# atonderski/future-object-detection

Hardware: AMD Instinct MI355X
Metric: frame-sequences/sec fwd+bwd, T=6 900x1600 (higher is better)
Workload: dtype bf16; 1 GPU; spatiotemporal ConditionalDETR (ResNet-50, 6 enc + 6 dec layers, 128 queries), T=6 frames 900x1600, batch 2/GPU, num_images K=5 (5 past frames live), random-init weights; step = forward (incl. Hungarian set loss, post-proc, AP bookkeeping) + backward + clip + AdamW; global_batch=2, frames=6, num_images=5, parallelism=dp1

## Files before the change

future-object-detection_amd/csrc/api.cpp:

```cpp
#include <stdarg.h>
#include <stdio.h>
#include <stdlib.h>
#include <string.h>

#include <mutex>

#include "../../include/fod.h"
#include "knobs.h"

static thread_local char g_err[512] = "";

void fod_set_error(const char* fmt, ...) {
  va_list ap;
  va_start(ap, fmt);
  vsnprintf(g_err, sizeof(g_err), fmt, ap);
  va_end(ap);
}

extern "C" size_t fod_last_error(char* buf, size_t cap) {
  const size_t n = strlen(g_err);
  if (buf && cap) {
    const size_t c = n < cap - 1 ? n : cap - 1;
    memcpy(buf, g_err, c);
    buf[c] = 0;
  }
  return n;
}

extern "C" int fod_abi_version(void) { return FOD_ABI_VERSION; }

extern "C" size_t fod_workspace_bytes(int kind) {
  switch (kind) {
    case FOD_WS_NT_SPLIT: return (size_t)FOD_NT_SPLIT_WS_FLOATS * sizeof(float);
    case FOD_WS_NT_SPLIT_TICKETS: return (size_t)FOD_NT_SPLIT_TICKETS * sizeof(unsigned);
    case FOD_WS_TN_PARTIALS: return FOD_TN_WS_BYTES;
    case FOD_WS_ATTN_SPLIT_PER_TILE: return (size_t)FOD_ATTN_SPLIT_WS_FLOATS_PER_TILE * sizeof(float);
    case FOD_WS_DET: return FOD_DET_WS_BYTES;
    case FOD_WS_TN_MULTI_DET: return FOD_TN_MULTI_DET_WS_BYTES;
    default: return 0;
  }
}

namespace {
struct KnobName {
  const char* name;
  int Knobs::*i;
  double Knobs::*d;
};
const KnobName KNOB_NAMES[] = {
    {"FOD_NT_SMALL", &Knobs::nt_small, nullptr},
    {"FOD_NT_NARROW", &Knobs::nt_narrow, nullptr},
    {"FOD_NT_SPLITK", &Knobs::nt_splitk, nullptr},
    {"FOD_NT_BIG", &Knobs::nt_big, nullptr},
    {"FOD_NT_BIG256", &Knobs::nt_big256, nullptr},
    {"FOD_NT_BIG_ILV", &Knobs::nt_big_ilv, nullptr},
    {"FOD_NT_BIG256_MINK", &Knobs::nt_big256_mink, nullptr},
    {"FOD_NT_BIG_MINK", &Knobs::nt_big_mink, nullptr},
    {"FOD_NT_BIG_MINN", &Knobs::nt_big_minn, nullptr},
    {"FOD_TN_SMALL", &Knobs::tn_small, nullptr},
    {"FOD_TN_BIG", &Knobs::tn_big, nullptr},
    {"FOD_TN_BIG_DENSE", &Knobs::tn_big_dense, nullptr},
    {"FOD_TN_BIG256", &Knobs::tn_big256, nullptr},
    {"FOD_TN_BIG_MIN", nullptr, &Knobs::tn_big_min},
    {"FOD_TN_BIG_SPLITS", &Knobs::tn_big_splits, nullptr},
    {"FOD_TN_WS", &Knobs::tn_ws, nullptr},
    {"FOD_TN_XCD", &Knobs::tn_xcd, nullptr},
    {"FOD_TN_ROWS", &Knobs::tn_rows, nullptr},
    {"FOD_ATTN_LDS", &Knobs::attn_lds, nullptr},
    {"FOD_ATTN_PF", &Knobs::attn_pf, nullptr},
    {"FOD_FP8_STAGE", &Knobs::fp8_stage, nullptr},
    {"FOD_LN_BWD_GROUPS", &Knobs::ln_bwd_groups, nullptr},
    {"FOD_BNK_VERSION", &Knobs::bnk_version, nullptr},
};

bool knob_parse(const KnobName& k, const char* text, Knobs& t) {
  char* end = nullptr;
  if (k.d) {
    const double v = strtod(text, &end);
    if (end == text || *end) return false;
    t.*k.d = v;
    return true;
  }
  if (Knobs{}.*k.i == Knobs::AUTO && !strcmp(text, "auto")) {
    t.*k.i = Knobs::AUTO;
    return true;
  }
  const long v = strtol(text, &end, 10);
  if (end == text || *end || v < 0 || v > 0x7FFFFFFF) return false;
  t.*k.i = (int)v;
  return true;
}

std::mutex g_knob_mutex;
Knobs& knob_table() {
  static Knobs table = [] {
    Knobs t;
    for (const KnobName& k : KNOB_NAMES)
      if (const char* text = getenv(k.name)) knob_parse(k, text, t);
    return t;
  }();
  return table;
}
const KnobName* knob_find(const char* name) {
  for (const KnobName& k : KNOB_NAMES)
    if (name && !strcmp(name, k.name)) return &k;
  fod_set_error("knob: unknown name %s", name ? name : "(null)");
  return nullptr;
}
}

Knobs fod_knobs() {
// ... 37 lines not shown
```

future-object-detection_amd/csrc/gemm_nt.hip:

```cpp
#include <stdlib.h>

#include <type_traits>

#include "common.h"
#include "gemm_nt.h"
#include "gemm_tn.h"

namespace {

using namespace fodnt;

template <typename T, int MODE, int NT, bool UTAP>
FOD_DEVINL void gemm_nt_body(const NtParams& p) {
  constexpr int VEC = Elem<T>::VEC;
  constexpr int BK = ROW_BYTES / (int)sizeof(T);
  constexpr int BN = 64 * NT;
  constexpr int KSTEPS = BK / 16;
  constexpr int BROWS = BN / 32;
  extern __shared__ __attribute__((aligned(16))) unsigned char smem[];
  unsigned char* sA = smem;
  unsigned char* sB = smem + 2 * BM * ROW_BYTES;

  const int tid = threadIdx.x;
  const int lane = tid & 63;
// ... 669 lines not shown
void fill_epilogue(NtParams& p, const fod_epilogue* e) {
  p.scale = e ? e->scale : nullptr;
  p.shift = e ? e->shift : nullptr;
  p.res = e ? e->residual : nullptr;
  p.ldr = e ? e->ld_residual : 0;
  p.res_row_mod = e ? e->residual_row_mod : 0;
  p.mask = e ? e->relu_mask : nullptr;
  p.ldmask = e ? e->ld_mask : 0;
  p.relu = e ? e->relu : 0;
  p.c_is_f32 = e ? e->out_f32 : 0;
  p.split_ws = e ? reinterpret_cast<float*>(e->split_ws) : nullptr;
  p.split_tickets = e ? reinterpret_cast<unsigned*>(e->split_tickets) : nullptr;
}

void decide_vec_epilogue(NtParams& p) {
  auto al = [](const void* q) { return ((uintptr_t)q % 16) == 0; };
  p.vec_epi = (p.N % 4 == 0) && (p.ldc % 4 == 0) && al(p.C) && (!p.scale || al(p.scale)) &&
              (!p.shift || al(p.shift)) && (!p.res || (p.ldr % 4 == 0 && al(p.res))) &&
              (!p.mask || (p.ldmask % 4 == 0 && al(p.mask)));
}

}

namespace fodnt {
namespace {
bool small_applies(int dtype, const NtParams& p, const Knobs& kn) {
  if (!kn.nt_small) return false;
  if (dtype != FOD_BF16 || !p.vec_epi) return false;
  const long blocks = (long)ceil_div(p.M, 64) * ceil_div(p.N, 64);
  if (blocks > 256) return false;
  if (p.res && ((long)(p.res_row_mod > 0 ? p.res_row_mod : p.M) * p.ldr + p.N) * 2 >= 0x7FFFFFF0L) return false;
  if (p.mask && ((long)p.M * p.ldmask + p.N) * 2 >= 0x7FFFFFF0L) return false;
  return true;
}

bool big256_applies(const NtParams& p, const Knobs& kn) {
  if (kn.nt_big256 == 0) return false;
  if (p.N < 256) return false;
  if (kn.nt_big256 == 2) return true;
  const long tiles = (long)ceil_div(p.M, BMB) * ceil_div(p.N, 256);
  return p.N % 256 == 0 && tiles >= 200;
}

bool big_applies(int mode, const NtParams& p, const Knobs& kn) {
  if (kn.nt_big == 0) return false;
  if (!p.vec_epi || p.a_seg_len || p.c_seg_cols) return false;
  if (mode == MODE_STEM) return false;
  if (mode != MODE_DENSE && (p.Cs % BKB_EL != 0 || p.K < BKB_EL)) return false;
  if (mode == MODE_DENSE && p.K % 8 != 0) return false;
  if (p.N % 4 != 0) return false;
  const long tiles = (long)ceil_div(p.M, BMB) * ceil_div(p.N, 128);
  if (kn.nt_big == 2) return true;
  if (mode != MODE_DENSE && p.K >= kn.nt_big256_mink && p.K < 1536 && big256_applies(p, kn)) return true;
  return p.K >= kn.nt_big_mink && p.N >= kn.nt_big_minn && tiles >= 200;
}
}

NtRoute route(int mode, int dtype, const NtParams& p, const Knobs& kn) {
  NtRoute r{};
  r.ksplit = 1;
  if (mode == MODE_DENSE && small_applies(dtype, p, kn)) {
    r.kernel = FOD_ROUTE_NT_SMALL;
    r.tile_n = 64;
    const long tiles = (long)ceil_div(p.N, 64) * ceil_div(p.M, 64);
    if (p.K >= 1024 && tiles <= 64 && kn.nt_splitk != 0) {
      const int cap = kn.nt_splitk > 1 ? (kn.nt_splitk < 8 ? kn.nt_splitk : 8) : 4;
      int ks = (int)(256 / tiles);
      if (ks > cap) ks = cap;
      if (ks > p.K / 256) ks = p.K / 256;
      r.wants_split_ws = ks > 1;
      if (ks > 1 && p.split_ws && p.split_tickets) r.ksplit = ks;
    }
    return r;
  }
  if (dtype == FOD_BF16 && big_applies(mode, p, kn)) {
    r.kernel = FOD_ROUTE_NT_BIG;
    const bool square = big256_applies(p, kn);
    r.tile_n = square ? 256 : 128;
    r.stages = square ? 2 : 3;
    r.interleave = kn.nt_big_ilv == Knobs::AUTO ? r.stages == 3 : kn.nt_big_ilv != 0;
    return r;
  }
  r.kernel = FOD_ROUTE_NT_128;
  r.stages = 2;
  const int narrow_below = kn.nt_narrow == Knobs::AUTO ? 320 : kn.nt_narrow;
  const long gy = ceil_div(p.M, BM);
  const long t_wide = gy * ceil_div(p.N, 128), t_narrow = gy * ceil_div(p.N, 64);
  const double fill_wide = (double)t_wide / (double)(ceil_div(t_wide, 512L) * 512L);
  const double fill_narrow = (double)t_narrow / (double)(ceil_div(t_narrow, 768L) * 768L);
  const bool narrow = p.N <= 64 || t_wide < narrow_below || (kn.nt_narrow == Knobs::AUTO && fill_narrow > 1.15 * fill_wide);
  r.tile_n = narrow ? 64 : 128;
  return r;
}
}

namespace {
int dense_params(NtParams& p, int dtype, const void* A, long lda, int a_row_mod, const void* B, long ldb, void* C,
                 long ldc, int M, int N, int K, const fod_epilogue* epi) {
  const int vec = dtype == FOD_BF16 ? 8 : 4;
  FOD_REQUIRE(M > 0 && N > 0 && K > 0, "gemm_nt: empty problem %d %d %d", M, N, K);
  FOD_REQUIRE(K % vec == 0 && lda % vec == 0 && ldb % vec == 0,
              "gemm_nt: K=%d lda=%ld ldb=%ld must be multiples of %d", K, lda, ldb, vec);
  FOD_REQUIRE(((uintptr_t)A % 16) == 0 && ((uintptr_t)B % 16) == 0, "gemm_nt: operands must be 16-byte aligned");
  p.A = A; p.B = B; p.C = C;
  p.lda = lda; p.ldb = ldb; p.ldc = ldc;
  p.M = M; p.N = N; p.K = K;
  p.a_row_mod = a_row_mod;
  fill_epilogue(p, epi);
  decide_vec_epilogue(p);
  const long esz = dtype == FOD_BF16 ? 2 : 4;
  const long a_rows = a_row_mod > 0 ? a_row_mod : M;
  const long ab = ((a_rows - 1) * lda + K) * esz, bb = ((long)(N - 1) * ldb + K) * esz;
  FOD_REQUIRE(ab < 0xFFFFFFF0L - 16 && bb < 0xFFFFFFF0L - 16, "gemm_nt: operand larger than 4 GiB");
  p.a_bytes = (unsigned)ab;
  p.b_bytes = (unsigned)bb;
  return FOD_OK;
}
}

extern "C" int fod_gemm_nt(int dtype, const void* A, long lda, int a_row_mod, const void* B, long ldb,
                           void* C, long ldc, int M, int N, int K, const fod_epilogue* epi,
                           hipStream_t stream) {
  FOD_REQUIRE(A && B && C, "gemm_nt: null operand");
  NtParams p{};
  if (int rc = dense_params(p, dtype, A, lda, a_row_mod, B, ldb, C, ldc, M, N, K, epi)) return rc;
  return launch<MODE_DENSE>(dtype, p, stream);
}

extern "C" int fod_gemm_nt_route(int dtype, long lda, int a_row_mod, long ldb, long ldc, int M, int N, int K,
                                 const fod_epilogue* epi, fod_nt_route* out) {
  FOD_REQUIRE(out && (dtype == FOD_BF16 || dtype == FOD_F32), "gemm_nt_route: bad args");
  NtParams p{};
  if (int rc = dense_params(p, dtype, nullptr, lda, a_row_mod, nullptr, ldb, nullptr, ldc, M, N, K, epi)) return rc;
// ... 228 lines not shown
```

future-object-detection_amd/csrc/gemm_nt_big.hip:

```cpp
#include <type_traits>

#include "common.h"
#include "gemm_nt.h"
#include "lds_dma.h"

namespace {

using namespace fodnt;

constexpr int A_DMA = BMB / 64;
template <int MODE, int BNB, int NSTAGE, bool ILV>
__global__ __launch_bounds__(512) void nt_big_kernel(const NtParams p) {
  constexpr int STAGE_BYTES = (BMB + BNB) * ROW_BYTES;
  constexpr int B_DMA = BNB / 64;
  constexpr int N_DMA = A_DMA + B_DMA;
  constexpr int NJ = BNB / 64;
  static_assert((BNB == 128 && NSTAGE == 3) || (BNB == 256 && NSTAGE == 2), "tile shapes: 256 x 128 x 3 stages, 256 x 256 x 2");
  typedef __bf16 T;
  constexpr unsigned ESZ = 2;
  constexpr unsigned BKB = BKB_EL * ESZ;
  constexpr int KSTEPS = BKB_EL / 16;
  extern __shared__ __attribute__((aligned(16))) unsigned char smem[];

  const int tid = threadIdx.x;
  const int lane = tid & 63;
  const int wave = __builtin_amdgcn_readfirstlane(tid >> 6);
  const int wm = wave >> 1, wn = wave & 1;
  const int xcd = blockIdx.x & 7, slot = blockIdx.x >> 3;
  const int nt_i = slot % p.gx;
  const int mt_i = (slot / p.gx) * 8 + xcd;
  if (mt_i >= p.gy) return;
  const int n0 = nt_i * BNB;
  const int m0 = mt_i * BMB;

  constexpr unsigned OOB = 0xFFFFFFF0u;
  const v4i rsA = make_rsrc(p.A, p.a_bytes), rsB = make_rsrc(p.B, p.b_bytes);
  const unsigned lds0 = (unsigned)(uintptr_t)(lds_ptr)smem;

  const int lrow = lane >> 3, lslot = lane & 7;
  unsigned a_base[A_DMA], a_cc[A_DMA];
  int a_h[A_DMA], a_w[A_DMA];
  int px_img = 0, px_h = 0, px_w = 0;
  if (MODE != MODE_DENSE) {
    const int mfirst = m0 + 8 * wave + lrow;
    const int hw = p.Hd * p.Wd;
    px_img = mfirst / hw;
    const int rem = mfirst - px_img * hw;
    px_h = rem / p.Wd;
    px_w = rem - px_h * p.Wd;
  }
#pragma unroll
  for (int i = 0; i < A_DMA; ++i) {
    const int row = 8 * (8 * i + wave) + lrow;
    const int m = m0 + row;
    const bool valid = m < p.M;
    a_cc[i] = (unsigned)((lslot ^ ((row >> 1) & 7)) * 16);
    if (MODE == MODE_DENSE) {
      const int r = p.a_row_mod > 0 ? (m % p.a_row_mod) : m;
      a_base[i] = valid ? (unsigned)((long)r * p.lda * (long)ESZ) + a_cc[i] : OOB;
      a_h[i] = a_w[i] = 0;
    } else {
      const int img = px_img, ph = px_h, pw = px_w;
      px_w += 64;
      while (px_w >= p.Wd) {
        px_w -= p.Wd;
        if (++px_h == p.Hd) {
          px_h = 0;
          ++px_img;
        }
      }
      a_base[i] = (unsigned)((long)img * p.Hs * p.Ws * p.Cs * (long)ESZ);
      if (MODE == MODE_CONV) {
        a_h[i] = valid ? ph * p.stride - p.pad : -(1 << 28);
        a_w[i] = pw * p.stride - p.pad;
      } else if (MODE == MODE_DGRAD_S2) {
        a_h[i] = valid ? ph + p.off_h : -(1 << 28);
        a_w[i] = pw + p.off_w;
      } else {
        a_h[i] = valid ? ph + p.pad : -(1 << 28);
        a_w[i] = pw + p.pad;
      }
      a_base[i] += ((unsigned)a_h[i] * (unsigned)p.Ws + (unsigned)a_w[i]) * (unsigned)p.Cs * ESZ + a_cc[i];
    }
  }
  unsigned b_base[B_DMA], b_cc[B_DMA];
#pragma unroll
  for (int i = 0; i < B_DMA; ++i) {
    const int row = 8 * (8 * i + wave) + lrow;
    const int n = n0 + row;
    b_cc[i] = (unsigned)((lslot ^ ((row >> 1) & 7)) * 16);
    b_base[i] = (n < p.N) ? (unsigned)((long)n * p.ldb * (long)ESZ) + b_cc[i] : OOB;
  }

  const int tap_w = MODE == MODE_DGRAD_S2 ? p.n_s : p.kw;
  const unsigned tap_row_skip = (unsigned)((p.Ws - tap_w) * p.Cs) * ESZ;
  const unsigned kb_row_skip = (unsigned)((2 * p.kw - 2 * tap_w) * p.Cs) * ESZ;
  const unsigned cs_b = (unsigned)p.Cs * ESZ;
  int tap_r = 0, tap_s = 0, tap_c = 0;
  unsigned tap_off = 0, tap_kb = 0;
  if (MODE == MODE_DGRAD_S2) tap_kb = (unsigned)((p.r_first * p.kw + p.s_first) * p.Cs) * ESZ;
  int next_kt = 0;

  struct TileCtx {
    int kt, r, s;
    unsigned kbyte, toff, kb, sA, sB;
// ... 27 lines not shown
    const bool tile_in = kt * BKB_EL < p.K;
    return TileCtx{kt, r, s, kbyte, toff, kb, sA, sB, tile_in};
  };
  auto issue_piece = [&](const TileCtx& c, auto pc_) {
    constexpr int pc = decltype(pc_)::value;
    if constexpr (pc < A_DMA) {
      constexpr int i = pc;
      unsigned off;
      if (MODE == MODE_DENSE) {
        const bool kin = (int)(c.kt * BKB_EL + (a_cc[i] >> 1)) < p.K;
        off = (kin && a_base[i] != OOB) ? a_base[i] + c.kbyte : OOB;
      } else {
        const int hs = MODE == MODE_CONV ? a_h[i] + c.r : a_h[i] - c.r;
        const int ws = MODE == MODE_CONV ? a_w[i] + c.s : a_w[i] - c.s;
        const bool ok = c.tile_in && (unsigned)hs < (unsigned)p.Hs && (unsigned)ws < (unsigned)p.Ws;
        off = ok ? (MODE == MODE_CONV ? a_base[i] + c.toff : a_base[i] - c.toff) : OOB;
      }
      dma16(rsA, c.sA + i * 8192, off);
    } else if constexpr (pc < A_DMA + B_DMA) {
      constexpr int i = pc - A_DMA;
      const bool kin = MODE == MODE_DENSE ? (int)(c.kt * BKB_EL + (b_cc[i] >> 1)) < p.K : c.tile_in;
      const unsigned off = (kin && b_base[i] != OOB) ? b_base[i] + c.kb : OOB;
      dma16(rsB, c.sB + i * 8192, off);
    }
  };
  auto issue_idx = [&](const TileCtx& c, int idx) {
    switch (idx) {
      case 0: issue_piece(c, std::integral_constant<int, 0>{}); break;
      case 1: issue_piece(c, std::integral_constant<int, 1>{}); break;
      case 2: issue_piece(c, std::integral_constant<int, 2>{}); break;
      case 3: issue_piece(c, std::integral_constant<int, 3>{}); break;
      case 4: issue_piece(c, std::integral_constant<int, 4>{}); break;
      case 5: issue_piece(c, std::integral_constant<int, 5>{}); break;
      case 6: issue_piece(c, std::integral_constant<int, 6>{}); break;
      case 7: issue_piece(c, std::integral_constant<int, 7>{}); break;
      default: break;
    }
  };
  auto issue_tile = [&](int stage) {
    const TileCtx c = begin_tile(stage);
#pragma unroll
    for (int idx = 0; idx < N_DMA; ++idx) issue_idx(c, idx);
  };

  f32x16 acc[2][NJ];
#pragma unroll
  for (int i = 0; i < 2; ++i)
#pragma unroll
    for (int j = 0; j < NJ; ++j)
#pragma unroll
      for (int r = 0; r < 16; ++r) acc[i][j][r] = 0.f;

  const int fr = lane & 31, fh = lane >> 5;
  auto read_frags = [&](const unsigned char* a_s, const unsigned char* b_s, int ks, Frag<T>* fa, Frag<T>* fb) {
#pragma unroll
    for (int i = 0; i < 2; ++i) {
      const int row = wm * 64 + i * 32 + fr;
      const uint4 v = *reinterpret_cast<const uint4*>(a_s + lds_off(row, 2 * ks + fh));
      __builtin_memcpy(&fa[i], &v, 16);
    }
#pragma unroll
    for (int j = 0; j < NJ; ++j) {
      const int row = wn * (BNB / 2) + j * 32 + fr;
      const uint4 v = *reinterpret_cast<const uint4*>(b_s + lds_off(row, 2 * ks + fh));
      __builtin_memcpy(&fb[j], &v, 16);
    }
  };
  static_assert(2 * KSTEPS >= N_DMA, "a tile's pieces are issued two per k-step");
  auto compute = [&](int stage, const TileCtx& fill) {
    const unsigned char* a_s = smem + stage * STAGE_BYTES;
    const unsigned char* b_s = a_s + BMB * ROW_BYTES;
    Frag<T> fa[2][2], fb[2][NJ];
    read_frags(a_s, b_s, 0, fa[0], fb[0]);
#pragma unroll
    for (int ks = 0; ks < KSTEPS; ++ks) {
      if (ks + 1 < KSTEPS) read_frags(a_s, b_s, ks + 1, fa[(ks + 1) & 1], fb[(ks + 1) & 1]);
#pragma unroll
      for (int i = 0; i < 2; ++i) {
#pragma unroll
        for (int j = 0; j < NJ; ++j) mma16(fa[ks & 1][i], fb[ks & 1][j], acc[i][j]);
        if constexpr (ILV) {
          __builtin_amdgcn_sched_barrier(0);
          issue_idx(fill, 2 * ks + i);
          __builtin_amdgcn_sched_barrier(0);
        }
      }
    }
  };

  auto wait_landed = [&](auto with_lgkm) {
    if constexpr (NSTAGE == 3) {
      static_assert(N_DMA == 6, "vmcnt immediate");
      if constexpr (decltype(with_lgkm)::value) asm volatile("s_waitcnt vmcnt(6) lgkmcnt(0)" ::: "memory");
      else asm volatile("s_waitcnt vmcnt(6)" ::: "memory");
    } else {
      if constexpr (decltype(with_lgkm)::value) asm volatile("s_waitcnt vmcnt(0) lgkmcnt(0)" ::: "memory");
      else asm volatile("s_waitcnt vmcnt(0)" ::: "memory");
    }
  };
  const int nkt = (p.K + BKB_EL - 1) / BKB_EL;
#pragma unroll
  for (int t = 0; t < NSTAGE - 1; ++t) issue_tile(t);
  wait_landed(std::false_type{});
  __builtin_amdgcn_s_barrier();
  int st_c = 0, st_i = NSTAGE - 1;
  for (int kt = 0; kt < nkt; ++kt) {
    const TileCtx fill = begin_tile(st_i);
    if constexpr (!ILV) {
#pragma unroll
      for (int idx = 0; idx < N_DMA; ++idx) issue_idx(fill, idx);
    }
    compute(st_c, fill);
    wait_landed(std::true_type{});
    __builtin_amdgcn_s_barrier();
    st_c = st_c == NSTAGE - 1 ? 0 : st_c + 1;
    st_i = st_i == NSTAGE - 1 ? 0 : st_i + 1;
  }
  asm volatile("s_waitcnt vmcnt(0)" ::: "memory");
  __builtin_amdgcn_s_barrier();

  const T* __restrict__ Rp = reinterpret_cast<const T*>(p.res);
  const T* __restrict__ Mp = reinterpret_cast<const T*>(p.mask);
  auto out_row = [&](int m) -> long {
    if (MODE != MODE_DGRAD_S2) return m;
    const int hw = p.Hd * p.Wd;
    const int img = m / hw;
    const int rem = m - img * hw;
    const int hq = rem / p.Wd;
    const int wq = rem - hq * p.Wd;
    return ((long)img * p.out_H + 2 * hq + p.par_h) * p.out_W + 2 * wq + p.par_w;
  };
  constexpr int HALVES = (BMB * BNB * 4 > NSTAGE * STAGE_BYTES) ? 2 : 1;
  constexpr int ROWS_H = BMB / HALVES;
  constexpr int CPR = BNB / 4;
  constexpr int RPP = 512 / CPR;
  constexpr int NPASS = ROWS_H / RPP;
  constexpr int PB = 8;
  const int cq = tid % CPR, rq = tid / CPR;
  const int n = n0 + cq * 4;
  const int nc = min(n, p.N - 4);
  float* sC = reinterpret_cast<float*>(smem);
  f32x4 sc = {1.f, 1.f, 1.f, 1.f}, sh = {0.f, 0.f, 0.f, 0.f};
  if (p.scale) sc = *reinterpret_cast<const f32x4*>(p.scale + nc);
  if (p.shift) sh = *reinterpret_cast<const f32x4*>(p.shift + nc);
  const bool full = m0 + BMB <= p.M && n0 + BNB <= p.N && !p.c_is_f32;
  int mh = 0;
  auto rows_out = [&](auto has_res, auto do_relu, auto has_mask, auto is_full) {
#pragma unroll
    for (int base = 0; base < NPASS; base += PB) {
      bf16x4_t rres[PB], rmsk[PB];
      f32x4 v[PB];
#pragma unroll
      for (int ps = 0; ps < PB; ++ps) {
        const long m = out_row(min(m0 + mh + rq + (base + ps) * RPP, p.M - 1));
        if constexpr (decltype(has_res)::value) {
          const long rm = p.res_row_mod > 0 ? (m % p.res_row_mod) : m;
          rres[ps] = *reinterpret_cast<const bf16x4_t*>(Rp + rm * p.ldr + nc);
        }
        if constexpr (decltype(has_mask)::value) rmsk[ps] = *reinterpret_cast<const bf16x4_t*>(Mp + m * p.ldmask + nc);
      }
#pragma unroll
      for (int ps = 0; ps < PB; ++ps)
        v[ps] = *reinterpret_cast<const f32x4*>(sC + (rq + (base + ps) * RPP) * BNB + cq * 4);
#pragma unroll
      for (int ps = 0; ps < PB; ++ps) {
        f32x4 w = v[ps] * sc + sh;
#pragma unroll
        for (int e = 0; e < 4; ++e) {
          if constexpr (decltype(has_res)::value) w[e] += (float)rres[ps][e];
          if constexpr (decltype(do_relu)::value) w[e] = fmaxf(w[e], 0.f);
          if constexpr (decltype(has_mask)::value) w[e] = ((float)rmsk[ps][e] > 0.f) ? w[e] : 0.f;
        }
        const int mt = m0 + mh + rq + (base + ps) * RPP;
        if constexpr (!decltype(is_full)::value) {
          if (mt >= p.M || n >= p.N) continue;
        }
        const long mo = out_row(mt);
        if (decltype(is_full)::value || !p.c_is_f32) {
          *reinterpret_cast<bf16x4_t*>(reinterpret_cast<__bf16*>(p.C) + mo * p.ldc + n) =
              bf16x4_t{(__bf16)w[0], (__bf16)w[1], (__bf16)w[2], (__bf16)w[3]};
        } else {
          *reinterpret_cast<f32x4*>(reinterpret_cast<float*>(p.C) + mo * p.ldc + n) = w;
        }
      }
    }
  };
  typedef std::true_type Y;
  typedef std::false_type N_;
  const bool R = Rp != nullptr, L = p.relu != 0, K = Mp != nullptr;
  auto pick = [&](auto is_full) {
    if (!R && !L && !K) rows_out(N_{}, N_{}, N_{}, is_full);
    else if (!R && L && !K) rows_out(N_{}, Y{}, N_{}, is_full);
    else if (R && L && !K) rows_out(Y{}, Y{}, N_{}, is_full);
    else if (R && !L && !K) rows_out(Y{}, N_{}, N_{}, is_full);
    else if (!R && !L && K) rows_out(N_{}, N_{}, Y{}, is_full);
    else if (R && !L && K) rows_out(Y{}, N_{}, Y{}, is_full);
    else if (!R && L && K) rows_out(N_{}, Y{}, Y{}, is_full);
    else rows_out(Y{}, Y{}, Y{}, is_full);
  };
#pragma unroll
  for (int h = 0; h < HALVES; ++h) {
    mh = h * ROWS_H;
    if (h > 0) __syncthreads();
    if (wm / (4 / HALVES) == h) {
#pragma unroll
      for (int i = 0; i < 2; ++i)
#pragma unroll
        for (int j = 0; j < NJ; ++j)
#pragma unroll
          for (int r = 0; r < 16; ++r)
            sC[((wm % (4 / HALVES)) * 64 + i * 32 + acc_row(r, lane)) * BNB + wn * (BNB / 2) + j * 32 + fr] = acc[i][j][r];
    }
    __syncthreads();
    if (full) pick(Y{});
    else pick(N_{});
  }
}

template <int MODE, int BNB, int NSTAGE, bool ILV>
int launch_big_ilv(const NtParams& q, hipStream_t stream) {
  static LdsLimitOnce lds_once;
  const size_t lds = (size_t)NSTAGE * (BMB + BNB) * ROW_BYTES;
  if (int rc = fod_lds_limit_once(lds_once, reinterpret_cast<const void*>(&nt_big_kernel<MODE, BNB, NSTAGE, ILV>), lds, "gemm_nt_big")) return rc;
  const dim3 grid(q.gx * ((q.gy + 7) / 8 * 8));
  hipLaunchKernelGGL((nt_big_kernel<MODE, BNB, NSTAGE, ILV>), grid, dim3(512), lds, stream, q);
  FOD_LAUNCH_CHECK();
  return FOD_OK;
}

template <int MODE>
int launch_big_mode(const NtParams& p, const NtRoute& r, hipStream_t stream) {
  NtParams q = p;
  q.gy = ceil_div(p.M, BMB);
  q.gx = ceil_div(p.N, r.tile_n);
  if (r.tile_n == 256)
    return r.interleave ? launch_big_ilv<MODE, 256, 2, true>(q, stream) : launch_big_ilv<MODE, 256, 2, false>(q, stream);
  return r.interleave ? launch_big_ilv<MODE, 128, 3, true>(q, stream) : launch_big_ilv<MODE, 128, 3, false>(q, stream);
}

}

namespace fodnt {

int launch_big(int mode, const NtParams& p, const NtRoute& r, hipStream_t stream) {
  switch (mode) {
    case MODE_DENSE: return launch_big_mode<MODE_DENSE>(p, r, stream);
    case MODE_CONV: return launch_big_mode<MODE_CONV>(p, r, stream);
    case MODE_DGRAD: return launch_big_mode<MODE_DGRAD>(p, r, stream);
    case MODE_DGRAD_S2: return launch_big_mode<MODE_DGRAD_S2>(p, r, stream);
    default: break;
  }
  fod_set_error("gemm_nt_big: unsupported mode %d", mode);
  return FOD_ERR_ARG;
}

}
```

future-object-detection_amd/csrc/knobs.h:

```cpp
#pragma once

struct Knobs {
  static constexpr int AUTO = -1;
  int nt_small = 1;
  int nt_narrow = AUTO;
  int nt_splitk = AUTO;
  int nt_big = 1;
  int nt_big256 = 1;
  int nt_big_ilv = AUTO;
  int nt_big256_mink = 128;
  int nt_big_mink = 1536;
  int nt_big_minn = 256;
  int tn_small = 1;
  int tn_big = 1;
  int tn_big_dense = 0;
  int tn_big256 = 0;
  double tn_big_min = 2.0e9;
  int tn_big_splits = 0;
  int tn_ws = 1;
  int tn_xcd = 1;
  int tn_rows = 0;
  int attn_lds = 8;
  int attn_pf = 1;
  int fp8_stage = 1;
  int ln_bwd_groups = 4;
  int bnk_version = 4;
};

Knobs fod_knobs();
```

future-object-detection_amd/future_od/native/lib.py:

```python
import contextlib
import ctypes as C
import os

_HERE = os.path.dirname(os.path.abspath(__file__))
LIB_PATH = os.path.normpath(os.path.join(_HERE, "..", "..", "lib", "libfod_hip.so"))
ABI_VERSION = 8

F32, BF16 = 0, 1
EW_ADD, EW_MUL, EW_RELU_MASK, EW_SCALE, EW_ADD3, EW_RELU, EW_COPY_B = range(7)


class FodError(RuntimeError):
    pass


class Epilogue(C.Structure):
    _fields_ = [("scale", C.c_void_p), ("shift", C.c_void_p), ("residual", C.c_void_p),
                ("ld_residual", C.c_long), ("residual_row_mod", C.c_int), ("relu_mask", C.c_void_p),
                ("ld_mask", C.c_long), ("relu", C.c_int), ("out_f32", C.c_int),
                ("split_ws", C.c_void_p), ("split_tickets", C.c_void_p)]


class ConvGeom(C.Structure):
    _fields_ = [("Nimg", C.c_int), ("H", C.c_int), ("W", C.c_int), ("Cin", C.c_int),
                ("Ho", C.c_int), ("Wo", C.c_int), ("Cout", C.c_int),
                ("kh", C.c_int), ("kw", C.c_int), ("stride", C.c_int), ("pad", C.c_int)]


class AttnShape(C.Structure):
    _fields_ = [("B", C.c_int), ("H", C.c_int), ("Tq", C.c_int), ("S", C.c_int),
                ("q_batch_stride", C.c_long), ("q_token_stride", C.c_long),
                ("k_batch_stride", C.c_long), ("k_token_stride", C.c_long),
                ("v_batch_stride", C.c_long), ("v_token_stride", C.c_long),
                ("o_batch_stride", C.c_long), ("o_token_stride", C.c_long),
                ("scale", C.c_float),
                ("k2_batch_stride", C.c_long), ("k2_token_stride", C.c_long),
                ("dk2_batch_stride", C.c_long), ("dk2_token_stride", C.c_long),
                ("drop_p", C.c_float), ("drop_seed", C.c_ulonglong), ("drop_seed_dev", C.c_void_p),
                ("split_ws", C.c_void_p), ("split_tickets", C.c_void_p), ("dq_scale", C.c_float)]


class PermuteJob(C.Structure):
    _fields_ = [("src", C.c_void_p), ("dst", C.c_void_p), ("scale", C.c_void_p),
                ("src_dtype", C.c_int), ("dst_dtype", C.c_int),
                ("d0", C.c_int), ("d1", C.c_int), ("d2", C.c_int),
                ("valid1", C.c_int), ("valid2", C.c_int), ("scale_axis", C.c_int),
                ("s0", C.c_long), ("s1", C.c_long), ("s2", C.c_long),
                ("t0", C.c_long), ("t1", C.c_long)]


class TnJob(C.Structure):
    _fields_ = [("G", C.c_void_p), ("X", C.c_void_p), ("dW", C.c_void_p), ("colsum", C.c_void_p),
                ("ldg", C.c_long), ("ldx", C.c_long), ("ldw", C.c_long),
                ("M", C.c_int), ("N1", C.c_int), ("K2", C.c_int), ("accumulate", C.c_int),
                ("g_seg_cols", C.c_int), ("chain", C.c_int), ("g_seg_stride", C.c_long),
                ("m_per_split", C.c_int), ("nsplit", C.c_int)]


class NtRoute(C.Structure):
    _fields_ = [("kernel", C.c_int), ("tile_n", C.c_int), ("stages", C.c_int), ("interleave", C.c_int),
                ("ksplit", C.c_int), ("wants_split_ws", C.c_int)]


class TnRoute(C.Structure):
    _fields_ = [("kernel", C.c_int), ("bi", C.c_int), ("bj", C.c_int), ("nsplit", C.c_int), ("m_per_split", C.c_int),
                ("xcd_order", C.c_int), ("uses_partials_ws", C.c_int)]


class AttnRoute(C.Structure):
    _fields_ = [("fwd", C.c_int), ("dq", C.c_int), ("dkv", C.c_int), ("fwd_waves", C.c_int), ("key_split", C.c_int),
                ("ksplit", C.c_int), ("kchunk", C.c_int)]


NT_SMALL, NT_128, NT_BIG = range(3)
TN_SMALL, TN_128, TN_BIG = range(3)
CONV_FWD, CONV_DGRAD, CONV_WGRAD = range(3)
ATTN_PLAIN, ATTN_LDS, ATTN_PREFETCH = range(3)

_i, _l, _f, _p = C.c_int, C.c_long, C.c_float, C.c_void_p
_EP, _CG, _AS = _p, _p, _p

SIGNATURES = {
    "fod_gemm_nt": [_i, _p, _l, _i, _p, _l, _p, _l, _i, _i, _i, _EP, _p],
    "fod_gemm_tn_acc": [_i, _p, _l, _p, _l, _p, _l, _i, _i, _i, _p, _p, _i, _p, C.c_size_t, _p],
    "fod_gemm_nt_grouped": [_i, _p, _l, _i, _l, _p, _l, _p, _l, _i, _l, _i, _i, _i, _EP, _i, _l, _p],
    "fod_gemm_nt_batched": [_i, _i, _p, _l, _l, _p, _l, _l, _p, _l, _l, _i, _i, _i, _EP, _l, _l, _l, _p],
    "fod_gemm_tn_grouped": [_i, _p, _l, _i, _l, _p, _l, _p, _l, _i, _i, _i, _p, _i, _p],
    "fod_gemm_tn_multi": [_p, _p, _p, _i, _p],
    "fod_gemm_tn_multi_long": [_p, _p, _p, _i, _p],
    "fod_tn_plan_long": [_i, _i, _p, _p],
    "fod_colsum_acc": [_i, _p, _l, _i, _i, _i, _p, _p],
    "fod_conv2d_fwd": [_i, _p, _p, _p, _CG, _EP, _p],
    "fod_conv2d_dgrad": [_i, _p, _p, _p, _CG, _EP, _p],
    "fod_conv_stem_fwd": [_i, _p, _p, _p, _i, _i, _i, _i, _i, _i, _EP, _p],
    "fod_stem_pool_fwd": [_i, _p, _p, _p, _p, _i, _i, _i, _i, _i, _i, _p],
    "fod_linear_add_norm_fwd": [_i, _p, _l, _p, _p, _p, _p, _p, _p, _p, _p, _p, _i, _i, _i, _f, _p, _p, _p, _p],
    "fod_linear_add_norm_bwd": [_i, _p, _p, _p, _p, _p, _p, _p, _p, _p, _p, _i, _i, _i, _p, _p, _p],
    "fod_clip_to_stem_layout": [_i, _i, _p, _p, _i, _i, _i, _i, _i, _i, _i, _l, _l, _p, _p, _p],
    "fod_clip_crop_resize": [_p, _p, _i, _i, _i, _i, _i, _i, _i, _l, _l, _p, _p, _p, _p],
    "fod_conv2d_wgrad_acc": [_i, _p, _p, _p, _CG, _p, _i, _p, C.c_size_t, _p],
    "fod_bottleneck_fused_fwd": [_i, _p, _p, _p, _p, _p, _p, _p, _p, _p, _p, _i, _i, _i, _i, _i, _i, _p],
    "fod_maxpool3x3s2": [_i, _p, _p, _i, _i, _i, _i, _i, _i, _p],
    "fod_dropout": [_i, _p, _p, _l, C.c_ulonglong, _p, _f, _p],
    "fod_multi_permute3": [_p, _p, _p, _i, _p],
    "fod_multi_permute_chunk": [],
    "fod_multi_permute_tiles": [_i, _i, _i, _l, _l, _l],
    "fod_nchw_to_nhwc": [_i, _p, _p, _i, _i, _i, _i, _i, _i, _l, _l, _p],
    "fod_u8_nchw_to_nhwc": [_i, _p, _p, _i, _i, _i, _i, _i, _i, _l, _l, _p, _p, _p],
    "fod_permute3_cast": [_i, _i, _p, _p, _i, _i, _i, _l, _l, _l, _i, _p, _i, _p],
    "fod_attn_fwd": [_i, _p, _p, _p, _p, _p, _p, _p, _AS, _p],
    "fod_attn_bwd": [_i, _p, _p, _p, _p, _p, _p, _p, _p, _p, _p, _p, _p, _p, _p, _AS, _p],
    "fod_attn_bwd_dq": [_i, _p, _p, _p, _p, _p, _p, _p, _p, _p, _p, _p, _AS, _p],
    "fod_attn_bwd_dkv_multi": [_i, _i, _p, _AS, _p],
    "fod_attn_fp8_pack_bytes": [_AS, _i, _p, _p],
# ... 176 lines not shown
```

include/fod.h:

```cpp
#ifndef FOD_H_
#define FOD_H_

#include <stddef.h>
#include <stdint.h>

#ifdef __cplusplus
extern "C" {
#endif

typedef struct ihipStream_t* fod_stream_t;

enum { FOD_F32 = 0, FOD_BF16 = 1 };
enum { FOD_OK = 0, FOD_ERR_ARG = 1, FOD_ERR_LAUNCH = 2, FOD_ERR_RUNTIME = 3 };

size_t fod_last_error(char* buf, size_t cap);
int fod_abi_version(void);
#define FOD_ABI_VERSION 8

int fod_knob_set(const char* name, const char* value);
int fod_knob_get(const char* name, char* out, size_t out_bytes);

enum { FOD_ROUTE_NT_SMALL = 0,
       FOD_ROUTE_NT_128 = 1,
       FOD_ROUTE_NT_BIG = 2 };
typedef struct fod_nt_route {
  int kernel;
  int tile_n;
  int stages;
  int interleave;
  int ksplit;
  int wants_split_ws;
} fod_nt_route;
enum { FOD_ROUTE_TN_SMALL = 0,
       FOD_ROUTE_TN_128 = 1,
       FOD_ROUTE_TN_BIG = 2 };
typedef struct fod_tn_route {
  int kernel;
  int bi, bj;
  int nsplit;
  int m_per_split;
  int xcd_order;
  int uses_partials_ws;
} fod_tn_route;

typedef struct fod_epilogue {
  const float* scale;
  const float* shift;
  const void* residual;
  long ld_residual;
  int residual_row_mod;
  const void* relu_mask;
  long ld_mask;
  int relu;
  int out_f32;
  void* split_ws;
  void* split_tickets;
} fod_epilogue;
#define FOD_NT_SPLIT_WS_FLOATS (64 * 8 * 4096)
#define FOD_NT_SPLIT_TICKETS 64
#define FOD_TN_WS_BYTES ((size_t)64 << 20)
enum { FOD_WS_NT_SPLIT = 0, FOD_WS_NT_SPLIT_TICKETS = 1, FOD_WS_TN_PARTIALS = 2, FOD_WS_ATTN_SPLIT_PER_TILE = 3,
       FOD_WS_DET = 4, FOD_WS_TN_MULTI_DET = 5 };
size_t fod_workspace_bytes(int kind);
#define FOD_DET_WS_BYTES ((size_t)16 << 20)
#define FOD_TN_MULTI_DET_WS_BYTES ((size_t)128 << 20)
#define FOD_TN_DET_MAX_SPLITS 4

int fod_gemm_nt(int dtype, const void* A, long lda, int a_row_mod, const void* B, long ldb, void* C,
                long ldc, int M, int N, int K, const fod_epilogue* epi, fod_stream_t stream);

int fod_gemm_nt_route(int dtype, long lda, int a_row_mod, long ldb, long ldc, int M, int N, int K,
                      const fod_epilogue* epi, fod_nt_route* out);

int fod_gemm_tn_acc(int dtype, const void* G, long ldg, const void* X, long ldx, float* dW, long ldw,
                    int M, int N1, int K2, const float* row_scale, float* colsum, int accumulate,
                    void* ws ,
                    size_t ws_bytes, fod_stream_t stream);
int fod_gemm_tn_route(int dtype, int M, int N1, int K2, long ldg, long ldx, long ldw, int has_row_scale,
                      int has_colsum, int det, size_t ws_bytes, fod_tn_route* out);

int fod_gemm_nt_grouped(int dtype, const void* A, long lda, int a_seg_len, long a_seg_stride, const void* B,
                        long ldb, void* C, long ldc, int c_seg_cols, long c_seg_stride, int M, int N, int K,
                        const fod_epilogue* epi,
                        int res_nseg, long res_seg_stride, fod_stream_t stream);
// ... 273 lines not shown
```

Before: 108.1 frame-sequences/s.

## Add slab-reuse 3x3 conv path to big NT GEMM and widen conv routing

Adds an optional slab form of the big NT GEMM kernel for stride-1 3x3 convs and dgrad. It loads one row slab of input per channel chunk into LDS and reuses it across the three horizontal taps by shifting rows, with boundary masking, instead of gathering im2col rows for every tap. The slab form sits behind a knob that defaults to off. Separately, a new default routing rule sends conv GEMMs with K ≥ 1152 and N ≥ 128 to the big kernel. This changes which kernel the mid-sized ResNet 3x3 convs use, and that kernel may not suit them.

```diff
diff --git a/future-object-detection_amd/csrc/api.cpp b/future-object-detection_amd/csrc/api.cpp
--- a/future-object-detection_amd/csrc/api.cpp
+++ b/future-object-detection_amd/csrc/api.cpp
@@ -57,6 +57,8 @@
     {"FOD_NT_BIG256_MINK", &Knobs::nt_big256_mink, nullptr},
     {"FOD_NT_BIG_MINK", &Knobs::nt_big_mink, nullptr},
     {"FOD_NT_BIG_MINN", &Knobs::nt_big_minn, nullptr},
+    {"FOD_NT_BIG_CONV_MINK", &Knobs::nt_big_conv_mink, nullptr},
+    {"FOD_NT_SLAB", &Knobs::nt_slab, nullptr},
     {"FOD_TN_SMALL", &Knobs::tn_small, nullptr},
     {"FOD_TN_BIG", &Knobs::tn_big, nullptr},
     {"FOD_TN_BIG_DENSE", &Knobs::tn_big_dense, nullptr},
diff --git a/future-object-detection_amd/csrc/gemm_nt.hip b/future-object-detection_amd/csrc/gemm_nt.hip
--- a/future-object-detection_amd/csrc/gemm_nt.hip
+++ b/future-object-detection_amd/csrc/gemm_nt.hip
@@ -745,7 +745,17 @@
   const long tiles = (long)ceil_div(p.M, BMB) * ceil_div(p.N, 128);
   if (kn.nt_big == 2) return true;
   if (mode != MODE_DENSE && p.K >= kn.nt_big256_mink && p.K < 1536 && big256_applies(p, kn)) return true;
+  if (mode != MODE_DENSE && p.K >= kn.nt_big_conv_mink && p.N >= 128 && tiles >= 200) return true;
   return p.K >= kn.nt_big_mink && p.N >= kn.nt_big_minn && tiles >= 200;
+}
+
+bool slab_applies(int mode, const NtParams& p, const Knobs& kn) {
+  if (kn.nt_slab == 0) return false;
+  if (mode != MODE_CONV && mode != MODE_DGRAD) return false;
+  if (p.kh != 3 || p.kw != 3 || p.stride != 1 || p.pad != 1 || p.Hs != p.Hd || p.Ws != p.Wd) return false;
+  if (p.Cs % BKB_EL != 0 || p.K != 9 * p.Cs) return false;
+  if (kn.nt_slab == 2) return true;
+  return (long)ceil_div(p.M, BMB) * ceil_div(p.N, 128) >= 200;
 }
 }
 
@@ -772,6 +782,7 @@
     r.tile_n = square ? 256 : 128;
     r.stages = square ? 2 : 3;
     r.interleave = kn.nt_big_ilv == Knobs::AUTO ? r.stages == 3 : kn.nt_big_ilv != 0;
+    r.slab = slab_applies(mode, p, kn);
     return r;
   }
   r.kernel = FOD_ROUTE_NT_128;
diff --git a/future-object-detection_amd/csrc/gemm_nt_big.hip b/future-object-detection_amd/csrc/gemm_nt_big.hip
--- a/future-object-detection_amd/csrc/gemm_nt_big.hip
+++ b/future-object-detection_amd/csrc/gemm_nt_big.hip
@@ -9,9 +9,20 @@
 using namespace fodnt;
 
 constexpr int A_DMA = BMB / 64;
-template <int MODE, int BNB, int NSTAGE, bool ILV>
+constexpr int nt_big_lds_bytes(int bnb, int nstage, bool slab) {
+  if (!slab) return nstage * (BMB + bnb) * ROW_BYTES;
+  const int loop = 2 * 33 * 1024 + 1024 + nstage * bnb * ROW_BYTES;
+  const int epi = BMB * bnb * 4 > 131072 ? BMB * bnb * 2 : BMB * bnb * 4;
+  return loop > epi ? loop : epi;
+}
+template <int MODE, int BNB, int NSTAGE, bool ILV, bool SLAB>
 __global__ __launch_bounds__(512) void nt_big_kernel(const NtParams p) {
-  constexpr int STAGE_BYTES = (BMB + BNB) * ROW_BYTES;
+  static_assert(!SLAB || MODE == MODE_CONV || MODE == MODE_DGRAD, "the slab form is for the stride-1 3x3 conv modes");
+  constexpr int SL_PIECES = 33, SL_DMA = 5;
+  constexpr int SL_BYTES = SL_PIECES * 1024, SL_DUMP = 2 * SL_BYTES, SL_B0 = SL_DUMP + 1024;
+  constexpr int STAGE_BYTES = SLAB ? BNB * ROW_BYTES : (BMB + BNB) * ROW_BYTES;
+  constexpr int LOOP_BYTES = SLAB ? SL_B0 + NSTAGE * STAGE_BYTES : NSTAGE * STAGE_BYTES;
+  constexpr int LDS_BYTES = nt_big_lds_bytes(BNB, NSTAGE, SLAB);
   constexpr int B_DMA = BNB / 64;
   constexpr int N_DMA = A_DMA + B_DMA;
   constexpr int NJ = BNB / 64;
@@ -41,7 +52,7 @@
   unsigned a_base[A_DMA], a_cc[A_DMA];
   int a_h[A_DMA], a_w[A_DMA];
   int px_img = 0, px_h = 0, px_w = 0;
-  if (MODE != MODE_DENSE) {
+  if (MODE != MODE_DENSE && !SLAB) {
     const int mfirst = m0 + 8 * wave + lrow;
     const int hw = p.Hd * p.Wd;
     px_img = mfirst / hw;
@@ -50,7 +61,7 @@
     px_w = rem - px_h * p.Wd;
   }
 #pragma unroll
-  for (int i = 0; i < A_DMA; ++i) {
+  for (int i = 0; i < (SLAB ? 0 : A_DMA); ++i) {
     const int row = 8 * (8 * i + wave) + lrow;
     const int m = m0 + row;
     const bool valid = m < p.M;
@@ -184,10 +195,10 @@
       for (int r = 0; r < 16; ++r) acc[i][j][r] = 0.f;
 
   const int fr = lane & 31, fh = lane >> 5;
-  auto read_frags = [&](const unsigned char* a_s, const unsigned char* b_s, int ks, Frag<T>* fa, Frag<T>* fb) {
+  auto read_frags = [&](const unsigned char* a_s, const unsigned char* b_s, int ks, Frag<T>* fa, Frag<T>* fb, int a_shift = 0) {
 #pragma unroll
     for (int i = 0; i < 2; ++i) {
-      const int row = wm * 64 + i * 32 + fr;
+      const int row = wm * 64 + i * 32 + fr + a_shift;
       const uint4 v = *reinterpret_cast<const uint4*>(a_s + lds_off(row, 2 * ks + fh));
       __builtin_memcpy(&fa[i], &v, 16);
     }
@@ -231,22 +242,210 @@
     }
   };
   const int nkt = (p.K + BKB_EL - 1) / BKB_EL;
-#pragma unroll
-  for (int t = 0; t < NSTAGE - 1; ++t) issue_tile(t);
-  wait_landed(std::false_type{});
-  __builtin_amdgcn_s_barrier();
-  int st_c = 0, st_i = NSTAGE - 1;
-  for (int kt = 0; kt < nkt; ++kt) {
-    const TileCtx fill = begin_tile(st_i);
-    if constexpr (!ILV) {
-#pragma unroll
-      for (int idx = 0; idx < N_DMA; ++idx) issue_idx(fill, idx);
-    }
-    compute(st_c, fill);
-    wait_landed(std::true_type{});
+  if constexpr (!SLAB) {
+#pragma unroll
+    for (int t = 0; t < NSTAGE - 1; ++t) issue_tile(t);
+    wait_landed(std::false_type{});
     __builtin_amdgcn_s_barrier();
-    st_c = st_c == NSTAGE - 1 ? 0 : st_c + 1;
-    st_i = st_i == NSTAGE - 1 ? 0 : st_i + 1;
+    int st_c = 0, st_i = NSTAGE - 1;
+    for (int kt = 0; kt < nkt; ++kt) {
+      const TileCtx fill = begin_tile(st_i);
+      if constexpr (!ILV) {
+#pragma unroll
+        for (int idx = 0; idx < N_DMA; ++idx) issue_idx(fill, idx);
+      }
+      compute(st_c, fill);
+      wait_landed(std::true_type{});
+      __builtin_amdgcn_s_barrier();
+      st_c = st_c == NSTAGE - 1 ? 0 : st_c + 1;
+      st_i = st_i == NSTAGE - 1 ? 0 : st_i + 1;
+    }
+  } else {
+    static_assert(2 * KSTEPS >= B_DMA + 3, "a tile's requests are issued two per k-step");
+    const unsigned csb = (unsigned)p.Cs * ESZ;
+    const int nslab = nkt / 3;
+    int sl_row[SL_DMA];
+    unsigned sl_rel[SL_DMA];
+#pragma unroll
+    for (int j = 0; j < SL_DMA; ++j) {
+      sl_row[j] = 8 * (wave + 8 * j) + lrow;
+      sl_rel[j] = (unsigned)sl_row[j] * csb + (unsigned)((lslot ^ ((sl_row[j] >> 1) & 7)) * 16);
+    }
+    unsigned a_ok[2], need = 0;
+    {
+      const int hw = p.Hd * p.Wd;
+#pragma unroll
+      for (int i = 0; i < 2; ++i) {
+        const int m = m0 + wm * 64 + i * 32 + fr;
+        const int img = m / hw;
+        const int rem = m - img * hw;
+        const int y = rem / p.Wd;
+        const int x = rem - y * p.Wd;
+        unsigned bits = 0;
+#pragma unroll
+        for (int r = 0; r < 3; ++r)
+#pragma unroll
+          for (int s2 = 0; s2 < 3; ++s2) {
+            const int dh = MODE == MODE_CONV ? r - 1 : 1 - r, dw = MODE == MODE_CONV ? s2 - 1 : 1 - s2;
+            const bool ok = m < p.M && (unsigned)(y + dh) < (unsigned)p.Hd && (unsigned)(x + dw) < (unsigned)p.Wd;
+            bits |= (ok ? 1u : 0u) << (3 * r + s2);
+          }
+        a_ok[i] = bits;
+      }
+#pragma unroll
+      for (int t = 0; t < 9; ++t)
+        if (__builtin_amdgcn_ballot_w64(((a_ok[0] & a_ok[1]) >> t & 1u) == 0u) != 0) need |= 1u << t;
+    }
+    int bq_t = 0, bq_r = 0, bq_c = 0, bq_s = 0;
+    int sq_g = 0, sq_r = 0, sq_c = 0;
+    struct BCtx {
+      unsigned kb, sB;
+      bool in;
+    };
+    struct SCtx {
+      unsigned base, sA;
+      int q0;
+      bool in;
+    };
+    auto begin_b = [&](int stage) {
+      const BCtx c{(unsigned)((3 * bq_r + bq_s) * p.Cs + bq_c) * ESZ, lds0 + (unsigned)(SL_B0 + stage * STAGE_BYTES + wave * 1024),
+                   bq_t < nkt};
+      ++bq_t;
+      if (++bq_s == 3) {
+        bq_s = 0;
+        bq_c += BKB_EL;
+        if (bq_c == p.Cs) {
+          bq_c = 0;
+          ++bq_r;
+        }
+      }
+      return c;
+    };
+    auto begin_slab = [&]() {
+      const int q0 = m0 + (MODE == MODE_CONV ? sq_r - 1 : 1 - sq_r) * p.Ws - 1;
+      const SCtx c{(unsigned)q0 * csb + (unsigned)sq_c * ESZ, lds0 + (unsigned)((sq_g & 1) * SL_BYTES), q0, sq_g < nslab};
+      ++sq_g;
+      sq_c += BKB_EL;
+      if (sq_c == p.Cs) {
+        sq_c = 0;
+        ++sq_r;
+      }
+      return c;
+    };
+    auto issue_b = [&](const BCtx& c, auto i_) {
+      constexpr int i = decltype(i_)::value;
+      dma16(rsB, c.sB + i * 8192, (c.in && b_base[i] != OOB) ? b_base[i] + c.kb : OOB);
+    };
+    auto issue_sl = [&](const SCtx& c, auto j_) {
+      constexpr int j = decltype(j_)::value;
+      const bool real = 8 * j < SL_PIECES - 8 || wave + 8 * j < SL_PIECES;
+      const bool ok = c.in && real && (unsigned)(c.q0 + sl_row[j]) < (unsigned)p.M;
+      dma16(rsA, real ? c.sA + (unsigned)((wave + 8 * j) * 1024) : lds0 + (unsigned)SL_DUMP, ok ? c.base + sl_rel[j] : OOB);
+    };
+    auto issue_slot = [&](const BCtx& b, const SCtx& sl, int s, int idx) {
+      switch (idx) {
+        case 0: issue_b(b, std::integral_constant<int, 0>{}); return;
+        case 1: issue_b(b, std::integral_constant<int, 1>{}); return;
+        case 2: if constexpr (B_DMA > 2) { issue_b(b, std::integral_constant<int, 2>{}); return; } break;
+        case 3: if constexpr (B_DMA > 2) { issue_b(b, std::integral_constant<int, 3>{}); return; } break;
+        default: break;
+      }
+      switch (3 * s + idx - B_DMA) {
+        case 0: issue_sl(sl, std::integral_constant<int, 0>{}); break;
+        case 1: issue_sl(sl, std::integral_constant<int, 1>{}); break;
+        case 3: issue_sl(sl, std::integral_constant<int, 2>{}); break;
+        case 4: issue_sl(sl, std::integral_constant<int, 3>{}); break;
+        case 5: issue_sl(sl, std::integral_constant<int, 4>{}); break;
+        default: break;
+      }
+    };
+    auto compute_slab = [&](const unsigned char* a_s, const unsigned char* b_s, int shift, int tbit, bool masked,
+                            const BCtx& b, const SCtx& sl, int s) {
+      Frag<T> fa[2][2], fb[2][NJ];
+      unsigned keep[2];
+#pragma unroll
+      for (int i = 0; i < 2; ++i) keep[i] = (unsigned)((int)(a_ok[i] << (31 - tbit)) >> 31);
+      read_frags(a_s, b_s, 0, fa[0], fb[0], shift);
+#pragma unroll
+      for (int ks = 0; ks < KSTEPS; ++ks) {
+        if (ks + 1 < KSTEPS) read_frags(a_s, b_s, ks + 1, fa[(ks + 1) & 1], fb[(ks + 1) & 1], shift);
+        if (masked) {
+#pragma unroll
+          for (int i = 0; i < 2; ++i) {
+            uint4 v;
+            __builtin_memcpy(&v, &fa[ks & 1][i], 16);
+            v.x &= keep[i]; v.y &= keep[i]; v.z &= keep[i]; v.w &= keep[i];
+            __builtin_memcpy(&fa[ks & 1][i], &v, 16);
+          }
+        }
+#pragma unroll
+        for (int i = 0; i < 2; ++i) {
+#pragma unroll
+          for (int j = 0; j < NJ; ++j) mma16(fa[ks & 1][i], fb[ks & 1][j], acc[i][j]);
+          if constexpr (ILV) {
+            __builtin_amdgcn_sched_barrier(0);
+            issue_slot(b, sl, s, 2 * ks + i);
+            __builtin_amdgcn_sched_barrier(0);
+          }
+        }
+      }
+    };
+    auto wait_tile = [&](int s) {
+      if constexpr (NSTAGE == 3) {
+        static_assert(B_DMA == 2, "vmcnt immediates");
+        if (s == 0) asm volatile("s_waitcnt vmcnt(4) lgkmcnt(0)" ::: "memory");
+        else if (s == 1) asm volatile("s_waitcnt vmcnt(7) lgkmcnt(0)" ::: "memory");
+        else asm volatile("s_waitcnt vmcnt(2) lgkmcnt(0)" ::: "memory");
+      } else {
+        if (s == 0) asm volatile("s_waitcnt vmcnt(2) lgkmcnt(0)" ::: "memory");
+        else if (s == 1) asm volatile("s_waitcnt vmcnt(3) lgkmcnt(0)" ::: "memory");
+        else asm volatile("s_waitcnt vmcnt(0) lgkmcnt(0)" ::: "memory");
+      }
+    };
+    {
+      const SCtx sl = begin_slab();
+      issue_sl(sl, std::integral_constant<int, 0>{});
+      issue_sl(sl, std::integral_constant<int, 1>{});
+      issue_sl(sl, std::integral_constant<int, 2>{});
+      issue_sl(sl, std::integral_constant<int, 3>{});
+      issue_sl(sl, std::integral_constant<int, 4>{});
+#pragma unroll
+      for (int t = 0; t < NSTAGE - 1; ++t) {
+        const BCtx b = begin_b(t);
+#pragma unroll
+        for (int idx = 0; idx < B_DMA; ++idx) issue_slot(b, sl, 2, idx);
+      }
+      if constexpr (NSTAGE == 3) asm volatile("s_waitcnt vmcnt(2)" ::: "memory");
+      else asm volatile("s_waitcnt vmcnt(0)" ::: "memory");
+      __builtin_amdgcn_s_barrier();
+    }
+    int st_c = 0, st_i = NSTAGE - 1;
+    int c_r = 0, c_c = 0;
+    for (int g = 0; g < nslab; ++g) {
+      const SCtx sl = begin_slab();
+      const unsigned char* a_s = smem + (g & 1) * SL_BYTES;
+#pragma unroll
+      for (int s = 0; s < 3; ++s) {
+        const BCtx b = begin_b(st_i);
+        if constexpr (!ILV) {
+#pragma unroll
+          for (int idx = 0; idx < B_DMA + 3; ++idx) issue_slot(b, sl, s, idx);
+        }
+        const unsigned char* b_s = smem + SL_B0 + st_c * STAGE_BYTES;
+        const int shift = MODE == MODE_CONV ? s : 2 - s;
+        const int tbit = 3 * c_r + s;
+        compute_slab(a_s, b_s, shift, tbit, ((need >> tbit) & 1u) != 0, b, sl, s);
+        wait_tile(s);
+        __builtin_amdgcn_s_barrier();
+        st_c = st_c == NSTAGE - 1 ? 0 : st_c + 1;
+        st_i = st_i == NSTAGE - 1 ? 0 : st_i + 1;
+      }
+      c_c += BKB_EL;
+      if (c_c == p.Cs) {
+        c_c = 0;
+        ++c_r;
+      }
+    }
   }
   asm volatile("s_waitcnt vmcnt(0)" ::: "memory");
   __builtin_amdgcn_s_barrier();
@@ -262,7 +461,8 @@
     const int wq = rem - hq * p.Wd;
     return ((long)img * p.out_H + 2 * hq + p.par_h) * p.out_W + 2 * wq + p.par_w;
   };
-  constexpr int HALVES = (BMB * BNB * 4 > NSTAGE * STAGE_BYTES) ? 2 : 1;
+  constexpr int HALVES = (BMB * BNB * 4 > LDS_BYTES) ? 2 : 1;
+  static_assert(LOOP_BYTES <= LDS_BYTES && BMB * BNB * 4 / HALVES <= LDS_BYTES, "the loop's LDS and the f32 tile fit");
   constexpr int ROWS_H = BMB / HALVES;
   constexpr int CPR = BNB / 4;
   constexpr int RPP = 512 / CPR;
@@ -349,15 +549,22 @@
   }
 }
 
-template <int MODE, int BNB, int NSTAGE, bool ILV>
+template <int MODE, int BNB, int NSTAGE, bool ILV, bool SLAB>
 int launch_big_ilv(const NtParams& q, hipStream_t stream) {
   static LdsLimitOnce lds_once;
-  const size_t lds = (size_t)NSTAGE * (BMB + BNB) * ROW_BYTES;
-  if (int rc = fod_lds_limit_once(lds_once, reinterpret_cast<const void*>(&nt_big_kernel<MODE, BNB, NSTAGE, ILV>), lds, "gemm_nt_big")) return rc;
+  const size_t lds = nt_big_lds_bytes(BNB, NSTAGE, SLAB);
+  if (int rc = fod_lds_limit_once(lds_once, reinterpret_cast<const void*>(&nt_big_kernel<MODE, BNB, NSTAGE, ILV, SLAB>), lds, "gemm_nt_big")) return rc;
   const dim3 grid(q.gx * ((q.gy + 7) / 8 * 8));
-  hipLaunchKernelGGL((nt_big_kernel<MODE, BNB, NSTAGE, ILV>), grid, dim3(512), lds, stream, q);
+  hipLaunchKernelGGL((nt_big_kernel<MODE, BNB, NSTAGE, ILV, SLAB>), grid, dim3(512), lds, stream, q);
   FOD_LAUNCH_CHECK();
   return FOD_OK;
+}
+
+template <int MODE, bool SLAB>
+int launch_big_tile(const NtParams& q, const NtRoute& r, hipStream_t stream) {
+  if (r.tile_n == 256)
+    return r.interleave ? launch_big_ilv<MODE, 256, 2, true, SLAB>(q, stream) : launch_big_ilv<MODE, 256, 2, false, SLAB>(q, stream);
+  return r.interleave ? launch_big_ilv<MODE, 128, 3, true, SLAB>(q, stream) : launch_big_ilv<MODE, 128, 3, false, SLAB>(q, stream);
 }
 
 template <int MODE>
@@ -365,9 +572,21 @@
   NtParams q = p;
   q.gy = ceil_div(p.M, BMB);
   q.gx = ceil_div(p.N, r.tile_n);
-  if (r.tile_n == 256)
-    return r.interleave ? launch_big_ilv<MODE, 256, 2, true>(q, stream) : launch_big_ilv<MODE, 256, 2, false>(q, stream);
-  return r.interleave ? launch_big_ilv<MODE, 128, 3, true>(q, stream) : launch_big_ilv<MODE, 128, 3, false>(q, stream);
+  if constexpr (MODE == MODE_CONV || MODE == MODE_DGRAD) {
+    if (r.slab) {
+      if (p.kh != 3 || p.kw != 3 || p.stride != 1 || p.pad != 1 || p.Hs != p.Hd || p.Ws != p.Wd || p.Cs % BKB_EL != 0 ||
+          p.K != 9 * p.Cs) {
+        fod_set_error("gemm_nt_big: the slab form takes 3x3 stride-1 pad-1 convolutions only");
+        return FOD_ERR_ARG;
+      }
+      return launch_big_tile<MODE, true>(q, r, stream);
+    }
+  }
+  if (r.slab) {
+    fod_set_error("gemm_nt_big: no slab form of mode %d", MODE);
+    return FOD_ERR_ARG;
+  }
+  return launch_big_tile<MODE, false>(q, r, stream);
 }
 
 }
diff --git a/future-object-detection_amd/csrc/knobs.h b/future-object-detection_amd/csrc/knobs.h
--- a/future-object-detection_amd/csrc/knobs.h
+++ b/future-object-detection_amd/csrc/knobs.h
@@ -11,6 +11,8 @@
   int nt_big256_mink = 128;
   int nt_big_mink = 1536;
   int nt_big_minn = 256;
+  int nt_big_conv_mink = 1152;
+  int nt_slab = 0;
   int tn_small = 1;
   int tn_big = 1;
   int tn_big_dense = 0;
diff --git a/future-object-detection_amd/future_od/native/lib.py b/future-object-detection_amd/future_od/native/lib.py
--- a/future-object-detection_amd/future_od/native/lib.py
+++ b/future-object-detection_amd/future_od/native/lib.py
@@ -4,7 +4,7 @@
 
 _HERE = os.path.dirname(os.path.abspath(__file__))
 LIB_PATH = os.path.normpath(os.path.join(_HERE, "..", "..", "lib", "libfod_hip.so"))
-ABI_VERSION = 8
+ABI_VERSION = 9
 
 F32, BF16 = 0, 1
 EW_ADD, EW_MUL, EW_RELU_MASK, EW_SCALE, EW_ADD3, EW_RELU, EW_COPY_B = range(7)
@@ -59,7 +59,7 @@
 
 class NtRoute(C.Structure):
     _fields_ = [("kernel", C.c_int), ("tile_n", C.c_int), ("stages", C.c_int), ("interleave", C.c_int),
-                ("ksplit", C.c_int), ("wants_split_ws", C.c_int)]
+                ("ksplit", C.c_int), ("wants_split_ws", C.c_int), ("slab", C.c_int)]
 
 
 class TnRoute(C.Structure):
diff --git a/include/fod.h b/include/fod.h
--- a/include/fod.h
+++ b/include/fod.h
@@ -15,7 +15,7 @@
 
 size_t fod_last_error(char* buf, size_t cap);
 int fod_abi_version(void);
-#define FOD_ABI_VERSION 8
+#define FOD_ABI_VERSION 9
 
 int fod_knob_set(const char* name, const char* value);
 int fod_knob_get(const char* name, char* out, size_t out_bytes);
@@ -30,6 +30,7 @@
   int interleave;
   int ksplit;
   int wants_split_ws;
+  int slab;
 } fod_nt_route;
 enum { FOD_ROUTE_TN_SMALL = 0,
        FOD_ROUTE_TN_128 = 1,
```

After: 108.1 frame-sequences/s. About the same (-0.0%).
